# qinzheng93/GeoTransformer

Measured on NVIDIA H100. Metric: point-cloud pairs/sec (3DMatch-shape synth), higher is better.
Workload: dtype f32

## Files before the change

geotransformer_b200/csrc/evaluation.cu:

```cuda
#include "common.cuh"
#include "geob200.h"

namespace geob200 {

__device__ __forceinline__ float sqn3(float x, float y, float z) { return __fadd_rn(__fadd_rn(__fmul_rn(x, x), __fmul_rn(y, y)), __fmul_rn(z, z)); }
__device__ __forceinline__ float sqd_mm(float ax, float ay, float az, float a2, float bx, float by, float bz, float b2) {
    const float xy = fmaf(az, bz, fmaf(ay, by, __fmul_rn(ax, bx)));
    return fmaxf(__fadd_rn(__fsub_rn(a2, __fmul_rn(2.0f, xy)), b2), 0.0f);
}
__device__ __forceinline__ void xform(const float* T, float x, float y, float z, float& ox, float& oy, float& oz) {
    ox = fmaf(z, T[2], fmaf(y, T[1], x * T[0])) + T[3];
    oy = fmaf(z, T[6], fmaf(y, T[5], x * T[4])) + T[7];
    oz = fmaf(z, T[10], fmaf(y, T[9], x * T[8])) + T[11];
}

__global__ void __launch_bounds__(256) nc_prepare_kernel(const float* __restrict__ ref_nodes, const float* __restrict__ src_nodes,
                                                         const float* __restrict__ ref_knn_pts, const float* __restrict__ src_knn_pts,
                                                         const unsigned char* __restrict__ ref_knn_masks,
                                                         const unsigned char* __restrict__ src_knn_masks, const __grid_constant__ Segs cl,
                                                         int B, int K, const float* __restrict__ T, float* __restrict__ nodes_out,
                                                         float* __restrict__ pts_out, float* __restrict__ max_dist, int* __restrict__ n_valid) {
    const int lane = threadIdx.x & 31;
    const int s = blockIdx.y;
    const int m = blockIdx.x * 8 + (threadIdx.x >> 5);
// ... 26 lines not shown
#pragma unroll
    for (int o = 16; o > 0; o >>= 1) nv += __shfl_xor_sync(0xffffffffu, nv, o);
    if (lane == 0) {
        nodes_out[3 * m] = nx; nodes_out[3 * m + 1] = ny; nodes_out[3 * m + 2] = nz;
        max_dist[m] = md;
        n_valid[m] = nv;
    }
}

__global__ void __launch_bounds__(256) nc_overlap_kernel(const float* __restrict__ ref_nodes, const float* __restrict__ src_nodes,
                                                         const float* __restrict__ ref_pts, const float* __restrict__ src_pts,
                                                         const unsigned char* __restrict__ ref_knn_masks,
                                                         const unsigned char* __restrict__ src_knn_masks,
                                                         const unsigned char* __restrict__ ref_masks, const unsigned char* __restrict__ src_masks,
                                                         const float* __restrict__ ref_max, const float* __restrict__ src_max,
                                                         const int* __restrict__ ref_nv, const int* __restrict__ src_nv,
                                                         const __grid_constant__ Segs R, const __grid_constant__ Segs Q,
                                                         const __grid_constant__ Segs NN, int K, float pos_radius,
                                                         float* __restrict__ overlap ) {
    const int b = blockIdx.y;
    const int M = R.count[b], N = Q.count[b];
    if ((int)blockIdx.x >= M) return;
    {
        const long long r = R.start[b], q = Q.start[b];
        ref_nodes += 3 * r; ref_pts += 3 * r * K; ref_max += r; ref_nv += r;
        if (ref_knn_masks != nullptr) ref_knn_masks += r * K;
        if (ref_masks != nullptr) ref_masks += r;
        src_nodes += 3 * q; src_pts += 3 * q * K; src_max += q; src_nv += q;
        if (src_knn_masks != nullptr) src_knn_masks += q * K;
        if (src_masks != nullptr) src_masks += q;
        overlap += NN.start[b];
    }
    extern __shared__ float sm[];
    float4* rp = reinterpret_cast<float4*>(sm);
    float4* sp = rp + K;
    int* rhit = reinterpret_cast<int*>(sp + K);
    int* shit = rhit + K;
    __shared__ int tot[2];
    const int m = blockIdx.x;
    const float r2 = pos_radius * pos_radius;
    for (int i = threadIdx.x; i < K; i += blockDim.x) {
        const float* p = ref_pts + ((long long)m * K + i) * 3;
        const bool ok = ref_knn_masks == nullptr || ref_knn_masks[(long long)m * K + i];
        rp[i] = make_float4(p[0], p[1], p[2], ok ? sqn3(p[0], p[1], p[2]) : -1.f);
    }
    const bool m_ok = ref_masks == nullptr || ref_masks[m];
    const float mx = ref_nodes[3 * m], my = ref_nodes[3 * m + 1], mz = ref_nodes[3 * m + 2];
    const float m2 = sqn3(mx, my, mz);
    __syncthreads();
    for (int n = 0; n < N; ++n) {
        float ov = 0.f;
        const bool n_ok = src_masks == nullptr || src_masks[n];
        const float sx = src_nodes[3 * n], sy = src_nodes[3 * n + 1], sz = src_nodes[3 * n + 2];
        const float dist = sqrtf(sqd_mm(mx, my, mz, m2, sx, sy, sz, sqn3(sx, sy, sz)));
        const bool inter = m_ok && n_ok && (ref_max[m] + src_max[n] + pos_radius - dist > 0.f);
        if (inter) {
            for (int j = threadIdx.x; j < K; j += blockDim.x) {
                const float* p = src_pts + ((long long)n * K + j) * 3;
                const bool ok = src_knn_masks == nullptr || src_knn_masks[(long long)n * K + j];
                sp[j] = make_float4(p[0], p[1], p[2], ok ? sqn3(p[0], p[1], p[2]) : -1.f);
                shit[j] = 0;
                rhit[j] = 0;
            }
            __syncthreads();
            for (int e = threadIdx.x; e < K * K; e += blockDim.x) {
                const int i = e / K, j = e % K;
                const float4 a = rp[i], b = sp[j];
                if (a.w >= 0.f && b.w >= 0.f && sqd_mm(a.x, a.y, a.z, a.w, b.x, b.y, b.z, b.w) < r2) { rhit[i] = 1; shit[j] = 1; }
            }
            __syncthreads();
            int cr = 0, cs = 0;
            for (int i = threadIdx.x; i < K; i += blockDim.x) { cr += rhit[i]; cs += shit[i]; }
            if (threadIdx.x == 0) { tot[0] = 0; tot[1] = 0; }
            __syncthreads();
            if (cr) atomicAdd(&tot[0], cr);
            if (cs) atomicAdd(&tot[1], cs);
            __syncthreads();
            ov = ((float)tot[0] / (float)ref_nv[m] + (float)tot[1] / (float)src_nv[n]) / 2.0f;
            __syncthreads();
        }
        if (threadIdx.x == 0) overlap[(long long)m * N + n] = ov;
    }
}

__global__ void __launch_bounds__(1024) nc_compact_kernel(const float* __restrict__ overlap, const __grid_constant__ Segs R,
                                                          const __grid_constant__ Segs Q, const __grid_constant__ Segs NN,
                                                          long long* __restrict__ idx, float* __restrict__ ov_out, int* __restrict__ count) {
    const int b = blockIdx.x;
    const int M = R.count[b], N = Q.count[b];
    overlap += NN.start[b]; idx += 2ll * NN.start[b]; ov_out += NN.start[b]; count += b;
    __shared__ int warp_tot[32];
    __shared__ int carry;
    const int lane = threadIdx.x & 31, warp = threadIdx.x >> 5;
    if (threadIdx.x == 0) carry = 0;
    __syncthreads();
    const long long total = (long long)M * N;
    for (long long base = 0; base < total; base += 4096) {
        const long long t0 = base + 4ll * threadIdx.x;
        float v[4];
        int f = 0;
#pragma unroll
        for (int u = 0; u < 4; ++u) {
            v[u] = (t0 + u < total) ? overlap[t0 + u] : 0.f;
            f += v[u] > 0.f ? 1 : 0;
        }
        int incl = f;
#pragma unroll
        for (int o = 1; o < 32; o <<= 1) {
            const int y = __shfl_up_sync(0xffffffffu, incl, o);
            if (lane >= o) incl += y;
        }
        if (lane == 31) warp_tot[warp] = incl;
        __syncthreads();
        int off = carry + incl - f;
// ... 434 lines not shown

size_t geob200_node_correspondences_batched_workspace_bytes(int64_t n_rows, int64_t n_products, int64_t k) {
    const size_t r = (size_t)n_rows;
    return align_up(12 * r, 256) + align_up(12 * r * (size_t)k, 256) + 2 * align_up(4 * r, 256) + align_up(4 * (size_t)n_products, 256) + 256;
}

int geob200_node_correspondences_batched(const float* ref_nodes, const float* src_nodes, const float* ref_knn_points,
                                         const float* src_knn_points, const uint8_t* ref_masks, const uint8_t* src_masks,
                                         const uint8_t* ref_knn_masks, const uint8_t* src_knn_masks, int64_t n_pairs, const int64_t* cloud_nodes,
                                         int64_t k, const float* transforms, float pos_radius, int64_t* corr_indices, float* corr_overlaps,
                                         int32_t* count, void* workspace, size_t workspace_bytes, void* stream) {
    cudaStream_t st = (cudaStream_t)stream;
    GEOB_REQUIRE(n_pairs > 0 && 2 * n_pairs <= GEOB_MAX_CLOUDS, "node_correspondences_batched: 1..%d pairs", GEOB_MAX_CLOUDS / 2);
    GEOB_REQUIRE(k > 0 && k <= 1024, "node_correspondences: bad shape");
    const int B = (int)n_pairs;
    Segs cl, Q, NN;
    if (segs_from_counts(&cl, 2 * n_pairs, cloud_nodes) || segs_from_counts(&Q, n_pairs, cloud_nodes + n_pairs)) return -1;
    const Segs R = segs_range(cl, 0, B);
    const int64_t ref_rows = cl.start[B], rows = (int64_t)cl.start[2 * B - 1] + cl.count[2 * B - 1];
    GEOB_REQUIRE(ref_rows > 0 && rows > ref_rows, "node_correspondences: bad shape");
    if (segs_products(&NN, R, Q)) return -1;
    const int64_t nn = (int64_t)NN.start[B - 1] + NN.count[B - 1];
    GEOB_REQUIRE(workspace_bytes >= geob200_node_correspondences_batched_workspace_bytes(rows, nn, k),
                 "node_correspondences_batched: workspace too small");
    Arena ar(workspace, workspace_bytes);
    float* cn = ar.take<float>(3 * rows);
    float* cp = ar.take<float>(3 * rows * k);
    float* cmax = ar.take<float>(rows);
    int* cnv = ar.take<int>(rows);
    float* overlap = ar.take<float>(nn);
    GEOB_REQUIRE(ar.ok(), "node_correspondences: workspace accounting error");
    nc_prepare_kernel<<<dim3((unsigned)((cl.max + 7) / 8 > 0 ? (cl.max + 7) / 8 : 1), 2 * B), 256, 0, st>>>(
        ref_nodes, src_nodes, ref_knn_points, src_knn_points, ref_knn_masks, src_knn_masks, cl, B, (int)k, transforms, cn, cp, cmax, cnv);
    const size_t smem = (size_t)k * (2 * sizeof(float4) + 2 * sizeof(int));
    if (R.max > 0)
        nc_overlap_kernel<<<dim3((unsigned)R.max, B), 256, smem, st>>>(cn, cn + 3 * ref_rows, cp, cp + 3 * ref_rows * k, ref_knn_masks,
                                                                      src_knn_masks, ref_masks, src_masks, cmax, cmax + ref_rows, cnv,
                                                                      cnv + ref_rows, R, Q, NN, (int)k, pos_radius, overlap);
    nc_compact_kernel<<<B, 1024, 0, st>>>(overlap, R, Q, NN, (long long*)corr_indices, corr_overlaps, count);
    GEOB_CHECK_LAUNCH();
    count_launches(3);
    return 0;
}

static int evaluate_impl(const int64_t* gt_idx, const float* gt_ov, const Segs& G, const int32_t* n_gt_dev, float acceptance_overlap,
                         const int64_t* ref_idx, const int64_t* src_idx, int64_t n_node_corr, const int32_t* n_node_corr_dev,
                         const float* ref_pts, const float* src_pts, int64_t n_corr, const int32_t* n_corr_dev, float acceptance_radius,
                         const float* gt_transform, const float* est_transform, int64_t transform_ld, const float* src_points,
                         const Segs& S0, int mode, float rmse_threshold, float rre_threshold, float rte_threshold, float* metrics,
                         int64_t metrics_ld, cudaStream_t st) {
    GEOB_REQUIRE(mode >= 0 && mode <= 2, "evaluate: mode must be 0 (3DMatch), 1 (KITTI) or 2 (ModelNet)");
    evaluate_kernel<<<G.n, 1024, 0, st>>>((const long long*)gt_idx, gt_ov, G, acceptance_overlap, (const long long*)ref_idx,
                                          (const long long*)src_idx, (int)n_node_corr, ref_pts, src_pts, (int)n_corr, acceptance_radius,
                                          gt_transform, est_transform, (int)transform_ld, src_points, S0, mode, rmse_threshold, rre_threshold,
                                          rte_threshold, metrics, (int)metrics_ld, n_gt_dev, n_node_corr_dev, n_corr_dev);
    GEOB_CHECK_LAUNCH();
    count_launches(1);
    return 0;
}

int geob200_evaluate_counts(const int64_t* gt_node_corr_indices, const float* gt_node_corr_overlaps, int64_t n_gt, const int32_t* n_gt_dev,
                            float acceptance_overlap, const int64_t* ref_node_corr_indices, const int64_t* src_node_corr_indices,
                            int64_t n_node_corr, const int32_t* n_node_corr_dev, const float* ref_corr_points, const float* src_corr_points,
                            int64_t n_corr, const int32_t* n_corr_dev, float acceptance_radius, const float* gt_transform,
                            const float* est_transform, const float* src_points, int64_t n_src_points, int mode, float rmse_threshold,
                            float rre_threshold, float rte_threshold, float* metrics, void* stream) {
    return evaluate_impl(gt_node_corr_indices, gt_node_corr_overlaps, segs_one(n_gt), n_gt_dev, acceptance_overlap, ref_node_corr_indices,
// ... 223 lines not shown
```

geotransformer_b200/csrc/matching.cu:

```cuda
#include "common.cuh"
#include "geob200.h"

namespace geob200 {

int segs_from_counts(Segs* s, int64_t n, const int64_t* counts) {
    if (n < 1 || n > GEOB_MAX_CLOUDS) { set_error("batch: 1..%d segments supported (got %lld)", GEOB_MAX_CLOUDS, (long long)n); return -1; }
    *s = Segs{};
    s->n = (int)n;
    int64_t o = 0;
    for (int i = 0; i < n; ++i) {
        if (counts[i] < 0) { set_error("batch: negative segment size"); return -1; }
        s->start[i] = (int)o;
        s->count[i] = (int)counts[i];
        s->max = s->max > (int)counts[i] ? s->max : (int)counts[i];
        o += counts[i];
    }
    if (o >= (1ll << 31)) { set_error("batch: too many rows (%lld)", (long long)o); return -1; }
    return 0;
}

Segs segs_one(int64_t count) {
    Segs s{};
    s.n = 1;
    s.max = (int)count;
// ... 93 lines not shown
    }
}

__global__ void __launch_bounds__(256) spm_colsum_kernel(const float* __restrict__ S, const int* __restrict__ rcount,
                                                         const int* __restrict__ scount, const __grid_constant__ Segs Q,
                                                         const __grid_constant__ Segs NN, float* __restrict__ colsum) {
    const int p = blockIdx.y;
    const int ld = Q.count[p];
    S += NN.start[p]; rcount += p; scount += p; colsum += Q.start[p];
    const int j = blockIdx.x * blockDim.x + threadIdx.x;
    if (j >= *scount) return;
    const int nr = *rcount;
    float s = 0.f;
    for (int i = 0; i < nr; ++i) s += S[(long long)i * ld + j];
    colsum[j] = s;
}

__global__ void __launch_bounds__(256) spm_dual_kernel(const float* __restrict__ S, const int* __restrict__ rcount,
                                                       const int* __restrict__ scount, const float* __restrict__ rowsum,
                                                       const float* __restrict__ colsum, const __grid_constant__ Segs R,
                                                       const __grid_constant__ Segs Q, const __grid_constant__ Segs NN, int dual,
                                                       float* __restrict__ flat) {
    const int p = blockIdx.y;
    const int ld = Q.count[p];
    S += NN.start[p]; flat += NN.start[p]; rcount += p; scount += p; rowsum += R.start[p]; colsum += Q.start[p];
    const int nr = *rcount, ns = *scount;
    const long long t = (long long)blockIdx.x * blockDim.x + threadIdx.x;
    if (t >= (long long)nr * ns) return;
    const int i = (int)(t / ns), j = (int)(t % ns);
    const float v = S[(long long)i * ld + j];
    flat[t] = dual ? (v / rowsum[i]) * (v / colsum[j]) : v;
}

template <int KMAX>
__global__ void __launch_bounds__(1024) topk_flat_kernel(const float* __restrict__ flat, const int* __restrict__ rcount,
                                                         const int* __restrict__ scount, int k_req, const int* __restrict__ ridx,
                                                         const int* __restrict__ sidx, const __grid_constant__ Segs R,
                                                         const __grid_constant__ Segs Q, const __grid_constant__ Segs NN,
                                                         long long* __restrict__ ref_out, long long* __restrict__ src_out,
                                                         float* __restrict__ score_out, int* __restrict__ k_out) {
    {
        const int p = blockIdx.y;
        flat += NN.start[p]; rcount += p; scount += p; ridx += R.start[p]; sidx += Q.start[p];
        ref_out += (long long)p * k_req; src_out += (long long)p * k_req; score_out += (long long)p * k_req; k_out += p;
    }
    __shared__ unsigned hist[256];
    __shared__ unsigned long long keys[KMAX];
    __shared__ unsigned prefix_s, kth_s;
    __shared__ int warp_tot[32], carry_gt, carry_eq;
    const int nr = *rcount, ns = *scount;
    const long long total = (long long)nr * ns;
    const int k = (int)min((long long)min(k_req, KMAX), total);
    const int lane = threadIdx.x & 31, warp = threadIdx.x >> 5;
    for (int i = k + threadIdx.x; i < k_req; i += blockDim.x) { ref_out[i] = -1; src_out[i] = -1; score_out[i] = 0.f; }
    if (k == 0) { if (threadIdx.x == 0) *k_out = 0; return; }
    unsigned prefix = 0, mask = 0;
    int remaining = k;
    for (int shift = 24; shift >= 0; shift -= 8) {
        for (int i = threadIdx.x; i < 256; i += blockDim.x) hist[i] = 0;
        __syncthreads();
        for (long long t = threadIdx.x; t < total; t += blockDim.x) {
            const unsigned b = __float_as_uint(flat[t]);
            if ((b & mask) == prefix) atomicAdd(&hist[(b >> shift) & 255u], 1u);
        }
        __syncthreads();
        if (threadIdx.x == 0) {
            int rem = remaining;
            int d = 255;
            for (; d > 0; --d) {
                if ((int)hist[d] >= rem) break;
                rem -= (int)hist[d];
            }
            prefix_s = prefix | ((unsigned)d << shift);
            kth_s = (unsigned)rem;
        }
        __syncthreads();
        prefix = prefix_s;
        remaining = (int)kth_s;
        mask |= (255u << shift);
        __syncthreads();
    }
    const unsigned thr = prefix;
    const int need_eq = remaining;
    const int n_gt = k - need_eq;
    if (threadIdx.x == 0) { carry_gt = 0; carry_eq = 0; }
    __syncthreads();
    for (long long base = 0; base < total; base += 1024) {
        const long long t = base + threadIdx.x;
        unsigned b = 0;
        if (t < total) b = __float_as_uint(flat[t]);
        const int fg = (t < total && b > thr) ? 1 : 0;
        const int fe = (t < total && b == thr) ? 1 : 0;
        const unsigned bg = __ballot_sync(0xffffffffu, fg), be = __ballot_sync(0xffffffffu, fe);
        const int pg = __popc(bg & ((1u << lane) - 1u)), pe = __popc(be & ((1u << lane) - 1u));
        if (lane == 0) warp_tot[warp] = (__popc(bg) << 16) | __popc(be);
        __syncthreads();
        int og = carry_gt, oe = carry_eq;
        for (int w = 0; w < warp; ++w) { og += warp_tot[w] >> 16; oe += warp_tot[w] & 0xFFFF; }
        const unsigned long long key = ((unsigned long long)b << 32) | (unsigned)(0xFFFFFFFFu - (unsigned)t);
        if (fg) keys[og + pg] = key;
        if (fe && oe + pe < need_eq) keys[n_gt + oe + pe] = key;
        __syncthreads();
        if (threadIdx.x == 0) {
            int tg = 0, te = 0;
            for (int w = 0; w < 32; ++w) { tg += warp_tot[w] >> 16; te += warp_tot[w] & 0xFFFF; }
            carry_gt += tg; carry_eq += te;
        }
        __syncthreads();
    }
    int n2 = 1;
    while (n2 < k) n2 <<= 1;
    for (int i = k + threadIdx.x; i < n2; i += blockDim.x) keys[i] = 0ull;
    __syncthreads();
    for (int kk = 2; kk <= n2; kk <<= 1)
        for (int j = kk >> 1; j > 0; j >>= 1) {
            for (int t = threadIdx.x; t < n2; t += blockDim.x) {
                const int p = t ^ j;
                if (p > t) {
                    const unsigned long long a = keys[t], b = keys[p];
                    const bool desc = ((t & kk) == 0);
                    if ((a < b) == desc) { keys[t] = b; keys[p] = a; }
                }
            }
            __syncthreads();
        }
    for (int i = threadIdx.x; i < k; i += blockDim.x) {
        const unsigned long long key = keys[i];
        const unsigned t = 0xFFFFFFFFu - (unsigned)(key & 0xFFFFFFFFull);
        ref_out[i] = ridx[t / ns];
        src_out[i] = sidx[t % ns];
        score_out[i] = __uint_as_float((unsigned)(key >> 32));
    }
    if (threadIdx.x == 0) *k_out = k;
}

__global__ void __launch_bounds__(256) gather_patches_kernel(const long long* __restrict__ corr, int P_all, const long long* __restrict__ knn,
                                                             const unsigned char* __restrict__ knn_masks, int K,
                                                             const float* __restrict__ pts, const __grid_constant__ Segs Nd,
                                                             const __grid_constant__ Segs Pt, long long* __restrict__ out_idx,
                                                             unsigned char* __restrict__ out_mask, float* __restrict__ out_pts) {
    const int s = blockIdx.y;
    const int P = corr != nullptr ? P_all : Nd.count[s];
// ... 214 lines not shown
            }
#pragma unroll
            for (int o = LPR / 2; o > 0; o >>= 1) mx = fmaxf(mx, __shfl_xor_sync(0xffffffffu, mx, o));
            float s = 0.f;
#pragma unroll
            for (int k = 0; k < NE; ++k) s += exp2f(t[k] - mx);
#pragma unroll
            for (int o = LPR / 2; o > 0; o >>= 1) s += __shfl_xor_sync(0xffffffffu, s, o);
            if (act && sub == 0) u[ij] = lmu2 - (log2f(s) + mx);
        }
        __syncthreads();
        {
            float t[NE], mx = -INFINITY;
#pragma unroll
            for (int k = 0; k < NE; ++k) {
                const int o = sub + LPR * k;
                t[k] = zc[k] + u[o < K1 ? o : 0];
                mx = fmaxf(mx, t[k]);
            }
#pragma unroll
            for (int o = LPR / 2; o > 0; o >>= 1) mx = fmaxf(mx, __shfl_xor_sync(0xffffffffu, mx, o));
            float s = 0.f;
#pragma unroll
            for (int k = 0; k < NE; ++k) s += exp2f(t[k] - mx);
#pragma unroll
            for (int o = LPR / 2; o > 0; o >>= 1) s += __shfl_xor_sync(0xffffffffu, s, o);
            if (act && sub == 0) v[ij] = lnu2 - (log2f(s) + mx);
        }
        __syncthreads();
    }
    for (int e = threadIdx.x; e < K1 * K1; e += blockDim.x) {
        const int i = e / K1, j = e % K1;
        out[(long long)p * K1 * K1 + e] = Z[i * ld + j] + (u[i] + v[j]) * LN2 - norm;
    }
}

template <int K, int LPR, int MAXT, int MINB>
__global__ void __launch_bounds__(MAXT, MINB) sinkhorn_bwd_kernel(const float* __restrict__ scores, const unsigned char* __restrict__ row_masks,
                                                           const unsigned char* __restrict__ col_masks, const float* __restrict__ alpha_p,
                                                           int iters, float inf, const float* __restrict__ grad,
                                                           float* __restrict__ hist, float* __restrict__ dscores,
                                                           float* __restrict__ dalpha_part) {
    constexpr int K1 = K + 1, ld = K1 | 1, NE = (K1 + LPR - 1) / LPR;
    extern __shared__ float sm[];
    float* Z = sm;
    float* D = Z + K1 * ld;
    float* pu = D + K1 * ld;
    float* pv = pu + K1;
    float* Lu = pv + K1;
    float* Lv = Lu + K1;
    float* gu = Lv + K1;
    float* gv = gu + K1;
    unsigned char* rmk = reinterpret_cast<unsigned char*>(gv + K1);
    unsigned char* cmk = rmk + K1;
    __shared__ int cnt_s[2];
    const int p = blockIdx.x;
    row_masks += (long long)p * K; col_masks += (long long)p * K;
    grad += (long long)p * K1 * K1;
    hist += (long long)p * 2 * iters * K1;
    dscores += (long long)p * K * K;
    if (threadIdx.x < 2) cnt_s[threadIdx.x] = 0;
    __syncthreads();
    {
        int cr = 0, cc = 0;
        for (int i = threadIdx.x; i < K; i += blockDim.x) { cr += row_masks[i] ? 1 : 0; cc += col_masks[i] ? 1 : 0; }
        if (cr) atomicAdd(&cnt_s[0], cr);
// ... 294 lines not shown
                                                              const int* __restrict__ off, const int* __restrict__ keys,
                                                              int* __restrict__ sorted) {
    const long long e = (long long)blockIdx.x * blockDim.x + threadIdx.x;
    if (e >= 2 * pr.per_side) return;
    const int row = pr.row_of(e, R, Q);
    if (row < 0) return;
    const int b = off[row], n = off[row + 1] - b;
    int rank = 0;
    for (int s = 0; s < n; ++s) rank += keys[b + s] < (int)e;
    sorted[b + rank] = (int)e;
}

__global__ void __launch_bounds__(128) patch_rows_reduce_kernel(const float* __restrict__ tmp, int C, const int* __restrict__ off,
                                                                const int* __restrict__ sorted, int n_ref_rows, float* __restrict__ gref,
                                                                float* __restrict__ gsrc) {
    const int row = blockIdx.x;
    float* out = row < n_ref_rows ? gref + (long long)row * C : gsrc + (long long)(row - n_ref_rows) * C;
    const int b = off[row], n = off[row + 1] - b;
    for (int c = threadIdx.x; c < C; c += blockDim.x) {
        float s = 0.f;
        for (int k = 0; k < n; ++k) s += tmp[(long long)sorted[b + k] * C + c];
        out[c] = s;
    }
}

}

using namespace geob200;

extern "C" {

size_t geob200_superpoint_matching_batched_workspace_bytes(int64_t n_rows, int64_t n_products, int64_t n_pairs) {
    const size_t r = (size_t)n_rows, nn = (size_t)n_products;
    return align_up(4 * r, 256) * 3 + align_up(4 * nn, 256) * 2 + align_up(8 * (size_t)n_pairs, 256) + 4096;
}

int geob200_superpoint_matching_batched(const float* ref_feats, const float* src_feats, int64_t channels, const uint8_t* ref_masks,
                                        const uint8_t* src_masks, int64_t n_pairs, const int64_t* cloud_nodes, int64_t num_correspondences,
                                        int dual, int64_t* corr_indices, float* corr_scores, int32_t* num_out, void* workspace,
                                        size_t workspace_bytes, void* stream) {
    cudaStream_t st = (cudaStream_t)stream;
    GEOB_REQUIRE(n_pairs > 0 && 2 * n_pairs <= GEOB_MAX_CLOUDS, "superpoint_matching_batched: 1..%d pairs", GEOB_MAX_CLOUDS / 2);
    GEOB_REQUIRE(num_correspondences > 0 && num_correspondences <= 1024, "superpoint_matching: num_correspondences must be in 1..1024");
    const int B = (int)n_pairs;
    Segs cl, Q, NN;
    if (segs_from_counts(&cl, 2 * n_pairs, cloud_nodes) || segs_from_counts(&Q, n_pairs, cloud_nodes + n_pairs)) return -1;
    const Segs R = segs_range(cl, 0, B);
    const int64_t ref_rows = cl.start[B], rows = (int64_t)cl.start[2 * B - 1] + cl.count[2 * B - 1];
    GEOB_REQUIRE(ref_rows > 0 && rows > ref_rows, "superpoint_matching: empty input");
    if (segs_products(&NN, R, Q)) return -1;
    const int64_t nn = (int64_t)NN.start[B - 1] + NN.count[B - 1];
    GEOB_REQUIRE(workspace_bytes >= geob200_superpoint_matching_batched_workspace_bytes(rows, nn, n_pairs),
                 "superpoint_matching_batched: workspace too small");
    const size_t smem = sizeof(float) * (channels + Q.max);
    GEOB_REQUIRE(smem <= 48 * 1024, "superpoint_matching: row does not fit shared memory");
    Arena ar(workspace, workspace_bytes);
    int* idx = ar.take<int>(rows);
    float* rowsum = ar.take<float>(rows);
    float* colsum = ar.take<float>(rows);
    float* S = ar.take<float>(nn);
    float* flat = ar.take<float>(nn);
    int* counts = ar.take<int>(2 * B);
    const int* ridx = idx;
    const int* sidx = idx + ref_rows;
    const dim3 g_rows((unsigned)(R.max > 0 ? R.max : 1), B), g_cols((unsigned)((Q.max + 255) / 256 > 0 ? (Q.max + 255) / 256 : 1), B),
        g_nn((unsigned)((NN.max + 255) / 256 > 0 ? (NN.max + 255) / 256 : 1), B);
    const int64_t k = num_correspondences;
    compact_masks_kernel<<<dim3(1, 2 * B), 1024, 0, st>>>(ref_masks, src_masks, cl, B, idx, counts);
    spm_scores_kernel<<<g_rows, 256, smem, st>>>(ref_feats, src_feats, (int)channels, ridx, counts, sidx, counts + B, R, Q, NN, S, rowsum);
    spm_colsum_kernel<<<g_cols, 256, 0, st>>>(S, counts, counts + B, Q, NN, colsum);
    spm_dual_kernel<<<g_nn, 256, 0, st>>>(S, counts, counts + B, rowsum, colsum, R, Q, NN, dual, flat);
    topk_flat_kernel<1024><<<dim3(1, B), 1024, 0, st>>>(flat, counts, counts + B, (int)k, ridx, sidx, R, Q, NN, (long long*)corr_indices,
                                                        (long long*)corr_indices + B * k, corr_scores, num_out);
    GEOB_CHECK_LAUNCH();
    count_launches(5);
    return 0;
}

int geob200_gather_patches_batched(const int64_t* corr_indices, int64_t n_corr, int64_t n_clouds, const int64_t* cloud_nodes,
                                   const int64_t* cloud_points, const int64_t* node_knn_indices, const uint8_t* node_knn_masks, int64_t k,
                                   const float* points, int64_t* out_indices, uint8_t* out_masks, float* out_points, void* stream) {
    Segs nd, pt;
    if (segs_from_counts(&nd, n_clouds, cloud_nodes) || segs_from_counts(&pt, n_clouds, cloud_points)) return -1;
    const int64_t per = corr_indices != nullptr ? n_corr : nd.max;
    if (per == 0) return 0;
    gather_patches_kernel<<<dim3((unsigned)((per * k + 255) / 256), (unsigned)n_clouds), 256, 0, (cudaStream_t)stream>>>(
        (const long long*)corr_indices, (int)n_corr, (const long long*)node_knn_indices, node_knn_masks, (int)k, points, nd, pt,
        (long long*)out_indices, out_masks, out_points);
    GEOB_CHECK_LAUNCH();
    count_launches(1);
    return 0;
}

int geob200_patch_scores_batched(const float* ref_feats, const float* src_feats, int64_t channels, int64_t n_pairs, const int64_t* cloud_points,
                                 const int64_t* ref_knn_indices, const int64_t* src_knn_indices, int64_t n_patches, int64_t k,
                                 float* scores, void* stream) {
    cudaStream_t st = (cudaStream_t)stream;
    GEOB_REQUIRE(n_pairs > 0 && 2 * n_pairs <= GEOB_MAX_CLOUDS, "patch_scores_batched: 1..%d pairs", GEOB_MAX_CLOUDS / 2);
    Segs R, Q;
    if (segs_from_counts(&R, n_pairs, cloud_points) || segs_from_counts(&Q, n_pairs, cloud_points + n_pairs)) return -1;
    if (n_patches == 0) return 0;
    const float div = sqrtf((float)channels);
    const dim3 grid((unsigned)n_patches, R.n);
#define LAUNCH_PS(TV) patch_scores_kernel<TV><<<grid, 256, 0, st>>>(ref_feats, src_feats, R, Q, (int)channels,                      \
                                                                    (const long long*)ref_knn_indices, (const long long*)src_knn_indices, div, scores)
    if (k == 64) LAUNCH_PS(4);
    else if (k == 128) LAUNCH_PS(8);
    else if (k == 32) LAUNCH_PS(2);
    else
        GEOB_REQUIRE(false, "patch_scores: num_points_in_patch=%lld unsupported (32, 64, 128)", (long long)k);
#undef LAUNCH_PS
    GEOB_CHECK_LAUNCH();
    count_launches(1);
    return 0;
}

int geob200_sinkhorn(const float* scores, const uint8_t* row_masks, const uint8_t* col_masks, const float* alpha,
                     int64_t n_patches, int64_t k, int64_t num_iterations, float inf, float* out, void* stream) {
    cudaStream_t st = (cudaStream_t)stream;
    if (n_patches == 0) return 0;
    const int K1 = (int)k + 1, ld = K1 | 1;
    const size_t smem = sizeof(float) * ((size_t)K1 * ld + 4 * K1);
    GEOB_REQUIRE(smem <= 200 * 1024, "sinkhorn: patch too large (k=%lld)", (long long)k);
    if (smem > 48 * 1024 && ensure_max_smem((const void*)sinkhorn_kernel)) return -1;
#define LAUNCH_SK_REG(LPRV, NEV, MT)                                                                                                  \
    {                                                                                                                            \
        if (smem > 48 * 1024 && ensure_max_smem((const void*)sinkhorn_reg_kernel<LPRV, NEV, MT>)) return -1;                         \
        const int threads = ((K1 * LPRV + 31) / 32) * 32;                                                                        \
        sinkhorn_reg_kernel<LPRV, NEV, MT><<<(unsigned)n_patches, threads, smem, st>>>(scores, row_masks, col_masks, alpha, (int)k,  \
                                                                                  (int)num_iterations, inf, out);               \
    }
    if (K1 <= 40) LAUNCH_SK_REG(8, 5, 320)
    else if (K1 <= 72) LAUNCH_SK_REG(8, 9, 576)
    else if (K1 <= 132) LAUNCH_SK_REG(4, 33, 544)
    else
        sinkhorn_kernel<<<(unsigned)n_patches, 1024, smem, st>>>(scores, row_masks, col_masks, alpha, (int)k, (int)num_iterations, inf, out);
#undef LAUNCH_SK_REG
    GEOB_CHECK_LAUNCH();
    count_launches(1);
    return 0;
}

size_t geob200_sinkhorn_backward_workspace_bytes(int64_t n_patches, int64_t k, int64_t num_iterations) {
    const size_t K1 = (size_t)k + 1;
    return align_up(4 * (size_t)n_patches * 2 * (size_t)num_iterations * K1, 256) + align_up(4 * (size_t)n_patches, 256) + 256;
}

int geob200_sinkhorn_backward(const float* scores, const uint8_t* row_masks, const uint8_t* col_masks, const float* alpha, int64_t n_patches,
                              int64_t k, int64_t num_iterations, float inf, const float* grad_out, float* grad_scores, float* grad_alpha,
                              void* workspace, size_t workspace_bytes, void* stream) {
    cudaStream_t st = (cudaStream_t)stream;
    GEOB_REQUIRE(n_patches >= 0 && n_patches <= 0x7fffffff, "sinkhorn_backward: bad patch count");
    GEOB_REQUIRE(k == 32 || k == 64 || k == 128, "sinkhorn_backward: k must be 32, 64 or 128, got %lld", (long long)k);
    GEOB_REQUIRE(num_iterations >= 1 && num_iterations <= 100000, "sinkhorn_backward: num_iterations must be in 1..100000");
    GEOB_REQUIRE(inf > 0.f, "sinkhorn_backward: inf must be positive");
    GEOB_REQUIRE(scores != nullptr && row_masks != nullptr && col_masks != nullptr && alpha != nullptr && grad_out != nullptr &&
                     grad_scores != nullptr && grad_alpha != nullptr,
                 "sinkhorn_backward: null pointer");
    GEOB_REQUIRE(workspace_bytes >= geob200_sinkhorn_backward_workspace_bytes(n_patches, k, num_iterations),
                 "sinkhorn_backward: workspace too small");
    const int K1 = (int)k + 1, ld = K1 | 1;
    const size_t smem = sizeof(float) * (2 * (size_t)K1 * ld + 6 * K1) + 2 * (size_t)K1;
    Arena ar(workspace, workspace_bytes);
    float* hist = ar.take<float>((size_t)n_patches * 2 * num_iterations * K1);
    float* part = ar.take<float>((size_t)n_patches);
    GEOB_REQUIRE(ar.ok(), "sinkhorn_backward: workspace accounting error");
    int n_launch = 1;
    if (n_patches > 0) {
#define LAUNCH_SK_BWD(KV, LPRV, MT, MB)                                                                                               \
    {                                                                                                                                 \
// ... 88 lines not shown
```

Measured before the change: 437.5.

## Warp-per-pair overlap, two-stage chunked top-k, and register Sinkhorn variant

Three independent changes. The node-overlap kernel now gives each warp its own source node, with per-warp shared buffers and ballot/popc reductions replacing block-wide syncs and shared atomics. Superpoint top-k becomes two stages: per-chunk radix selection of candidates across many blocks, then a final single-block select over the candidates, instead of one block scanning all scores. A new Sinkhorn kernel for small patches spreads each line over 8 lanes holding two lines per group, using ex2.approx, and needs more workspace and shared memory.

```diff
diff --git a/geotransformer_b200/csrc/evaluation.cu b/geotransformer_b200/csrc/evaluation.cu
--- a/geotransformer_b200/csrc/evaluation.cu
+++ b/geotransformer_b200/csrc/evaluation.cu
@@ -82,11 +82,9 @@
         overlap += NN.start[b];
     }
     extern __shared__ float sm[];
+    const int lane = threadIdx.x & 31, warp = threadIdx.x >> 5, nw = blockDim.x >> 5;
     float4* rp = reinterpret_cast<float4*>(sm);
-    float4* sp = rp + K;
-    int* rhit = reinterpret_cast<int*>(sp + K);
-    int* shit = rhit + K;
-    __shared__ int tot[2];
+    float4* sp = rp + K + warp * K;
     const int m = blockIdx.x;
     const float r2 = pos_radius * pos_radius;
     for (int i = threadIdx.x; i < K; i += blockDim.x) {
@@ -98,38 +96,37 @@
     const float mx = ref_nodes[3 * m], my = ref_nodes[3 * m + 1], mz = ref_nodes[3 * m + 2];
     const float m2 = sqn3(mx, my, mz);
     __syncthreads();
-    for (int n = 0; n < N; ++n) {
+    for (int n = warp; n < N; n += nw) {
         float ov = 0.f;
         const bool n_ok = src_masks == nullptr || src_masks[n];
         const float sx = src_nodes[3 * n], sy = src_nodes[3 * n + 1], sz = src_nodes[3 * n + 2];
         const float dist = sqrtf(sqd_mm(mx, my, mz, m2, sx, sy, sz, sqn3(sx, sy, sz)));
         const bool inter = m_ok && n_ok && (ref_max[m] + src_max[n] + pos_radius - dist > 0.f);
         if (inter) {
-            for (int j = threadIdx.x; j < K; j += blockDim.x) {
+            for (int j = lane; j < K; j += 32) {
                 const float* p = src_pts + ((long long)n * K + j) * 3;
                 const bool ok = src_knn_masks == nullptr || src_knn_masks[(long long)n * K + j];
                 sp[j] = make_float4(p[0], p[1], p[2], ok ? sqn3(p[0], p[1], p[2]) : -1.f);
-                shit[j] = 0;
-                rhit[j] = 0;
             }
-            __syncthreads();
-            for (int e = threadIdx.x; e < K * K; e += blockDim.x) {
-                const int i = e / K, j = e % K;
-                const float4 a = rp[i], b = sp[j];
-                if (a.w >= 0.f && b.w >= 0.f && sqd_mm(a.x, a.y, a.z, a.w, b.x, b.y, b.z, b.w) < r2) { rhit[i] = 1; shit[j] = 1; }
+            __syncwarp();
+            unsigned rhit = 0;
+            int cs = 0;
+            for (int j = 0; j < K; ++j) {
+                const float4 b = sp[j];
+                bool hit = false;
+                for (int q = 0, i = lane; i < K; ++q, i += 32) {
+                    const float4 a = rp[i];
+                    if (a.w >= 0.f && b.w >= 0.f && sqd_mm(a.x, a.y, a.z, a.w, b.x, b.y, b.z, b.w) < r2) { rhit |= 1u << q; hit = true; }
+                }
+                cs += __any_sync(0xffffffffu, hit) ? 1 : 0;
             }
-            __syncthreads();
-            int cr = 0, cs = 0;
-            for (int i = threadIdx.x; i < K; i += blockDim.x) { cr += rhit[i]; cs += shit[i]; }
-            if (threadIdx.x == 0) { tot[0] = 0; tot[1] = 0; }
-            __syncthreads();
-            if (cr) atomicAdd(&tot[0], cr);
-            if (cs) atomicAdd(&tot[1], cs);
-            __syncthreads();
-            ov = ((float)tot[0] / (float)ref_nv[m] + (float)tot[1] / (float)src_nv[n]) / 2.0f;
-            __syncthreads();
-        }
-        if (threadIdx.x == 0) overlap[(long long)m * N + n] = ov;
+            int cr = __popc(rhit);
+#pragma unroll
+            for (int o = 16; o > 0; o >>= 1) cr += __shfl_xor_sync(0xffffffffu, cr, o);
+            ov = ((float)cr / (float)ref_nv[m] + (float)cs / (float)src_nv[n]) / 2.0f;
+            __syncwarp();
+        }
+        if (lane == 0) overlap[(long long)m * N + n] = ov;
     }
 }
 
@@ -630,7 +627,8 @@
     GEOB_REQUIRE(ar.ok(), "node_correspondences: workspace accounting error");
     nc_prepare_kernel<<<dim3((unsigned)((cl.max + 7) / 8 > 0 ? (cl.max + 7) / 8 : 1), 2 * B), 256, 0, st>>>(
         ref_nodes, src_nodes, ref_knn_points, src_knn_points, ref_knn_masks, src_knn_masks, cl, B, (int)k, transforms, cn, cp, cmax, cnv);
-    const size_t smem = (size_t)k * (2 * sizeof(float4) + 2 * sizeof(int));
+    const size_t smem = (size_t)k * sizeof(float4) * (1 + 256 / 32);
+    if (smem > 48 * 1024 && ensure_max_smem((const void*)nc_overlap_kernel)) return -1;
     if (R.max > 0)
         nc_overlap_kernel<<<dim3((unsigned)R.max, B), 256, smem, st>>>(cn, cn + 3 * ref_rows, cp, cp + 3 * ref_rows * k, ref_knn_masks,
                                                                       src_knn_masks, ref_masks, src_masks, cmax, cmax + ref_rows, cnv,
diff --git a/geotransformer_b200/csrc/matching.cu b/geotransformer_b200/csrc/matching.cu
--- a/geotransformer_b200/csrc/matching.cu
+++ b/geotransformer_b200/csrc/matching.cu
@@ -149,82 +149,131 @@
     flat[t] = dual ? (v / rowsum[i]) * (v / colsum[j]) : v;
 }
 
-template <int KMAX>
-__global__ void __launch_bounds__(1024) topk_flat_kernel(const float* __restrict__ flat, const int* __restrict__ rcount,
-                                                         const int* __restrict__ scount, int k_req, const int* __restrict__ ridx,
-                                                         const int* __restrict__ sidx, const __grid_constant__ Segs R,
-                                                         const __grid_constant__ Segs Q, const __grid_constant__ Segs NN,
-                                                         long long* __restrict__ ref_out, long long* __restrict__ src_out,
-                                                         float* __restrict__ score_out, int* __restrict__ k_out) {
-    {
-        const int p = blockIdx.y;
-        flat += NN.start[p]; rcount += p; scount += p; ridx += R.start[p]; sidx += Q.start[p];
-        ref_out += (long long)p * k_req; src_out += (long long)p * k_req; score_out += (long long)p * k_req; k_out += p;
-    }
-    __shared__ unsigned hist[256];
-    __shared__ unsigned long long keys[KMAX];
-    __shared__ unsigned prefix_s, kth_s;
-    __shared__ int warp_tot[32], carry_gt, carry_eq;
-    const int nr = *rcount, ns = *scount;
-    const long long total = (long long)nr * ns;
-    const int k = (int)min((long long)min(k_req, KMAX), total);
-    const int lane = threadIdx.x & 31, warp = threadIdx.x >> 5;
-    for (int i = k + threadIdx.x; i < k_req; i += blockDim.x) { ref_out[i] = -1; src_out[i] = -1; score_out[i] = 0.f; }
-    if (k == 0) { if (threadIdx.x == 0) *k_out = 0; return; }
+constexpr int TOPK_CHUNK = 4096;
+constexpr int TOPK_KMAX = 1024;
+
+struct TopkShared {
+    unsigned hist[256];
+    unsigned prefix, kth;
+    int warp_tot[32], carry_gt, carry_eq;
+};
+
+template <typename Get>
+__device__ __forceinline__ void topk_threshold(int n, int k, Get b_of, TopkShared& sh, unsigned& thr, int& need_eq) {
     unsigned prefix = 0, mask = 0;
     int remaining = k;
     for (int shift = 24; shift >= 0; shift -= 8) {
-        for (int i = threadIdx.x; i < 256; i += blockDim.x) hist[i] = 0;
-        __syncthreads();
-        for (long long t = threadIdx.x; t < total; t += blockDim.x) {
-            const unsigned b = __float_as_uint(flat[t]);
-            if ((b & mask) == prefix) atomicAdd(&hist[(b >> shift) & 255u], 1u);
+        for (int i = threadIdx.x; i < 256; i += blockDim.x) sh.hist[i] = 0;
+        __syncthreads();
+        for (int t = threadIdx.x; t < n; t += blockDim.x) {
+            const unsigned b = b_of(t);
+            if ((b & mask) == prefix) atomicAdd(&sh.hist[(b >> shift) & 255u], 1u);
         }
         __syncthreads();
         if (threadIdx.x == 0) {
             int rem = remaining;
             int d = 255;
             for (; d > 0; --d) {
-                if ((int)hist[d] >= rem) break;
-                rem -= (int)hist[d];
+                if ((int)sh.hist[d] >= rem) break;
+                rem -= (int)sh.hist[d];
             }
-            prefix_s = prefix | ((unsigned)d << shift);
-            kth_s = (unsigned)rem;
-        }
-        __syncthreads();
-        prefix = prefix_s;
-        remaining = (int)kth_s;
+            sh.prefix = prefix | ((unsigned)d << shift);
+            sh.kth = (unsigned)rem;
+        }
+        __syncthreads();
+        prefix = sh.prefix;
+        remaining = (int)sh.kth;
         mask |= (255u << shift);
         __syncthreads();
     }
-    const unsigned thr = prefix;
-    const int need_eq = remaining;
-    const int n_gt = k - need_eq;
-    if (threadIdx.x == 0) { carry_gt = 0; carry_eq = 0; }
-    __syncthreads();
-    for (long long base = 0; base < total; base += 1024) {
-        const long long t = base + threadIdx.x;
-        unsigned b = 0;
-        if (t < total) b = __float_as_uint(flat[t]);
-        const int fg = (t < total && b > thr) ? 1 : 0;
-        const int fe = (t < total && b == thr) ? 1 : 0;
+    thr = prefix;
+    need_eq = remaining;
+}
+
+template <typename Get, typename Emit>
+__device__ __forceinline__ void topk_sweep(int n, unsigned thr, int need_eq, Get b_of, TopkShared& sh, Emit emit) {
+    const int lane = threadIdx.x & 31, warp = threadIdx.x >> 5, nw = blockDim.x >> 5;
+    if (threadIdx.x == 0) { sh.carry_gt = 0; sh.carry_eq = 0; }
+    __syncthreads();
+    for (int base = 0; base < n; base += blockDim.x) {
+        const int t = base + threadIdx.x;
+        const unsigned b = t < n ? b_of(t) : 0u;
+        const int fg = (t < n && b > thr) ? 1 : 0;
+        const int fe = (t < n && b == thr) ? 1 : 0;
         const unsigned bg = __ballot_sync(0xffffffffu, fg), be = __ballot_sync(0xffffffffu, fe);
         const int pg = __popc(bg & ((1u << lane) - 1u)), pe = __popc(be & ((1u << lane) - 1u));
-        if (lane == 0) warp_tot[warp] = (__popc(bg) << 16) | __popc(be);
-        __syncthreads();
-        int og = carry_gt, oe = carry_eq;
-        for (int w = 0; w < warp; ++w) { og += warp_tot[w] >> 16; oe += warp_tot[w] & 0xFFFF; }
-        const unsigned long long key = ((unsigned long long)b << 32) | (unsigned)(0xFFFFFFFFu - (unsigned)t);
-        if (fg) keys[og + pg] = key;
-        if (fe && oe + pe < need_eq) keys[n_gt + oe + pe] = key;
+        if (lane == 0) sh.warp_tot[warp] = (__popc(bg) << 16) | __popc(be);
+        __syncthreads();
+        int og = sh.carry_gt, oe = sh.carry_eq;
+        for (int w = 0; w < warp; ++w) { og += sh.warp_tot[w] >> 16; oe += sh.warp_tot[w] & 0xFFFF; }
+        if (fg || (fe && oe + pe < need_eq)) emit(og + pg + min(oe + pe, need_eq), t, b);
         __syncthreads();
         if (threadIdx.x == 0) {
             int tg = 0, te = 0;
-            for (int w = 0; w < 32; ++w) { tg += warp_tot[w] >> 16; te += warp_tot[w] & 0xFFFF; }
-            carry_gt += tg; carry_eq += te;
-        }
-        __syncthreads();
-    }
+            for (int w = 0; w < nw; ++w) { tg += sh.warp_tot[w] >> 16; te += sh.warp_tot[w] & 0xFFFF; }
+            sh.carry_gt += tg; sh.carry_eq += te;
+        }
+        __syncthreads();
+    }
+}
+
+__global__ void __launch_bounds__(256) topk_chunk_kernel(const float* __restrict__ flat, const int* __restrict__ rcount,
+                                                         const int* __restrict__ scount, int k_req, const __grid_constant__ Segs NN,
+                                                         unsigned* __restrict__ cand_b, unsigned* __restrict__ cand_t) {
+    const int p = blockIdx.y, c = blockIdx.x;
+    const long long total = (long long)rcount[p] * scount[p];
+    const int k = (int)min((long long)min(k_req, TOPK_KMAX), total);
+    const long long first = (long long)c * TOPK_CHUNK;
+    if (first >= total) return;
+    const int n = (int)min((long long)TOPK_CHUNK, total - first);
+    flat += NN.start[p] + first;
+    const long long slot = ((long long)NN.start[p] / TOPK_CHUNK + p + c) * k_req;
+    cand_b += slot; cand_t += slot;
+    __shared__ unsigned vals[TOPK_CHUNK];
+    __shared__ TopkShared sh;
+    for (int i = threadIdx.x; i < n; i += blockDim.x) vals[i] = __float_as_uint(flat[i]);
+    if (n <= k) {
+        for (int i = threadIdx.x; i < n; i += blockDim.x) { cand_b[i] = vals[i]; cand_t[i] = (unsigned)(first + i); }
+        return;
+    }
+    __syncthreads();
+    const auto b_of = [&](int t) { return vals[t]; };
+    unsigned thr;
+    int need_eq;
+    topk_threshold(n, k, b_of, sh, thr, need_eq);
+    topk_sweep(n, thr, need_eq, b_of, sh, [&](int slot, int t, unsigned b) { cand_b[slot] = b; cand_t[slot] = (unsigned)(first + t); });
+}
+
+template <int KMAX>
+__global__ void __launch_bounds__(1024) topk_flat_kernel(const unsigned* __restrict__ cand_b, const unsigned* __restrict__ cand_t,
+                                                         const int* __restrict__ rcount, const int* __restrict__ scount, int k_req,
+                                                         const int* __restrict__ ridx, const int* __restrict__ sidx,
+                                                         const __grid_constant__ Segs R, const __grid_constant__ Segs Q,
+                                                         const __grid_constant__ Segs NN, long long* __restrict__ ref_out,
+                                                         long long* __restrict__ src_out, float* __restrict__ score_out,
+                                                         int* __restrict__ k_out) {
+    {
+        const int p = blockIdx.y;
+        const long long slot = ((long long)NN.start[p] / TOPK_CHUNK + p) * k_req;
+        cand_b += slot; cand_t += slot; rcount += p; scount += p; ridx += R.start[p]; sidx += Q.start[p];
+        ref_out += (long long)p * k_req; src_out += (long long)p * k_req; score_out += (long long)p * k_req; k_out += p;
+    }
+    __shared__ unsigned long long keys[KMAX];
+    __shared__ TopkShared sh;
+    const int nr = *rcount, ns = *scount;
+    const long long total = (long long)nr * ns;
+    const int k = (int)min((long long)min(k_req, KMAX), total);
+    for (int i = k + threadIdx.x; i < k_req; i += blockDim.x) { ref_out[i] = -1; src_out[i] = -1; score_out[i] = 0.f; }
+    if (k == 0) { if (threadIdx.x == 0) *k_out = 0; return; }
+    const long long chunks = (total + TOPK_CHUNK - 1) / TOPK_CHUNK;
+    const int n = (int)((chunks - 1) * k_req + min((long long)k, total - (chunks - 1) * TOPK_CHUNK));
+    const auto b_of = [&](int t) { return cand_b[t]; };
+    unsigned thr;
+    int need_eq;
+    topk_threshold(n, k, b_of, sh, thr, need_eq);
+    topk_sweep(n, thr, need_eq, b_of, sh, [&](int slot, int t, unsigned b) {
+        keys[slot] = ((unsigned long long)b << 32) | (unsigned)(0xFFFFFFFFu - cand_t[t]);
+    });
     int n2 = 1;
     while (n2 < k) n2 <<= 1;
     for (int i = k + threadIdx.x; i < n2; i += blockDim.x) keys[i] = 0ull;
@@ -505,6 +554,158 @@
     for (int e = threadIdx.x; e < K1 * K1; e += blockDim.x) {
         const int i = e / K1, j = e % K1;
         out[(long long)p * K1 * K1 + e] = Z[i * ld + j] + (u[i] + v[j]) * LN2 - norm;
+    }
+}
+
+__device__ __forceinline__ float ex2_ftz(float x) {
+    float y;
+    asm("ex2.approx.ftz.f32 %0, %1;" : "=f"(y) : "f"(x));
+    return y;
+}
+
+template <int NE>
+struct SkLines {
+    static constexpr int PS = ((NE + 3) / 4 * 4) | 4;
+    static constexpr int ZS = ((2 * NE + 3) / 4 * 4) % 8 ? (2 * NE + 3) / 4 * 4 : (2 * NE + 3) / 4 * 4 + 4;
+};
+
+template <int NE, int NL>
+__device__ __forceinline__ void sinkhorn2_half_step(const float (&z)[2][NE], const float* __restrict__ pin, float* __restrict__ pout,
+                                                    int sub, const int (&line)[2], const bool (&own)[2], const float (&marg)[2]) {
+    constexpr int PS = SkLines<NE>::PS;
+    constexpr float LOG2E = 1.4426950408889634f;
+    float pv[NE];
+    {
+        const float* src = pin + sub * PS;
+#pragma unroll
+        for (int k = 0; k + 4 <= NE; k += 4) {
+            const float4 q = *reinterpret_cast<const float4*>(src + k);
+            pv[k] = q.x; pv[k + 1] = q.y; pv[k + 2] = q.z; pv[k + 3] = q.w;
+        }
+#pragma unroll
+        for (int k = NE / 4 * 4; k < NE; ++k) pv[k] = src[k];
+    }
+    float t[NL][NE], mx[NL], s[NL];
+#pragma unroll
+    for (int l = 0; l < NL; ++l) {
+        mx[l] = -INFINITY;
+#pragma unroll
+        for (int k = 0; k < NE; ++k) {
+            t[l][k] = __fadd_rn(z[l][k], pv[k]);
+            mx[l] = fmaxf(mx[l], t[l][k]);
+        }
+    }
+#pragma unroll
+    for (int o = 4; o > 0; o >>= 1)
+#pragma unroll
+        for (int l = 0; l < NL; ++l) mx[l] = fmaxf(mx[l], __shfl_xor_sync(0xffffffffu, mx[l], o));
+#pragma unroll
+    for (int l = 0; l < NL; ++l) {
+        s[l] = ex2_ftz(__fsub_rn(t[l][0], mx[l]));
+#pragma unroll
+        for (int k = 1; k < NE; ++k) s[l] = __fadd_rn(s[l], ex2_ftz(__fsub_rn(t[l][k], mx[l])));
+    }
+#pragma unroll
+    for (int o = 4; o > 0; o >>= 1)
+#pragma unroll
+        for (int l = 0; l < NL; ++l) s[l] = __fadd_rn(s[l], __shfl_xor_sync(0xffffffffu, s[l], o));
+    const bool second = NL == 2 && sub == 1;
+    if (sub < NL && (second ? own[1] : own[0])) {
+        const float ss = second ? s[NL - 1] : s[0], m = second ? mx[NL - 1] : mx[0];
+        const int i = second ? line[1] : line[0];
+        pout[(i & 7) * PS + (i >> 3)] = __fmaf_rn(second ? marg[1] : marg[0], LOG2E, -(log2f(ss) + m));
+    }
+}
+
+template <int NE, int MAXT, int MINB>
+__global__ void __launch_bounds__(MAXT, MINB) sinkhorn_reg2_kernel(const float* __restrict__ scores, const unsigned char* __restrict__ row_masks,
+                                                                   const unsigned char* __restrict__ col_masks, const float* __restrict__ alpha_p,
+                                                                   int K, int iters, float inf, float* __restrict__ out) {
+    constexpr int PS = SkLines<NE>::PS, ZS = SkLines<NE>::ZS;
+    extern __shared__ float sm[];
+    __shared__ __align__(16) float up[8 * PS], vp[8 * PS];
+    __shared__ float norm_s;
+    __shared__ int cnt_s[2];
+    const int K1 = K + 1;
+    const int ld = K1 | 1;
+    const int H = (K1 + 1) >> 1;
+    float* Z = sm;
+    float* zcs = sm + ((K1 * ld + 3) & ~3) + threadIdx.x * ZS;
+    const int p = blockIdx.x;
+    const float alpha = *alpha_p;
+    constexpr float LOG2E = 1.4426950408889634f, LN2 = 0.6931471805599453f;
+    if (threadIdx.x < 2) cnt_s[threadIdx.x] = 0;
+    for (int i = threadIdx.x; i < 8 * PS; i += blockDim.x) { up[i] = 0.f; vp[i] = 0.f; }
+    __syncthreads();
+    {
+        int cr = 0, cc = 0;
+        for (int i = threadIdx.x; i < K; i += blockDim.x) { cr += row_masks[(long long)p * K + i] ? 1 : 0; cc += col_masks[(long long)p * K + i] ? 1 : 0; }
+        if (cr) atomicAdd(&cnt_s[0], cr);
+        if (cc) atomicAdd(&cnt_s[1], cc);
+    }
+    __syncthreads();
+    const float nvr = (float)cnt_s[0], nvc = (float)cnt_s[1];
+    if (threadIdx.x == 0) norm_s = -logf(nvr + nvc);
+    __syncthreads();
+    const float norm = norm_s;
+    for (int e = threadIdx.x; e < K1 * K1; e += blockDim.x) {
+        const int i = e / K1, j = e % K1;
+        float z = (i < K && j < K) ? scores[((long long)p * K + i) * K + j] : alpha;
+        const bool rm = (i < K) && !row_masks[(long long)p * K + i];
+        const bool cm = (j < K) && !col_masks[(long long)p * K + j];
+        if (rm || cm) z = -inf;
+        Z[i * ld + j] = z;
+    }
+    __syncthreads();
+    const int g = threadIdx.x >> 3, sub = threadIdx.x & 7;
+    const bool two = ((threadIdx.x >> 5) << 2) + H < K1;
+    int line[2];
+    bool own[2];
+    float zr[2][NE], mu[2], nu[2];
+#pragma unroll
+    for (int l = 0; l < 2; ++l) {
+        const int i = g + l * H;
+        own[l] = (l == 0 ? g < H : true) && i < K1;
+        line[l] = own[l] ? i : K1 - 1;
+        const int ij = line[l];
+#pragma unroll
+        for (int k = 0; k < NE; ++k) {
+            const int o = sub + 8 * k;
+            zr[l][k] = (o < K1) ? __fmul_rn(Z[ij * ld + o], LOG2E) : -INFINITY;
+            zcs[l * NE + k] = (o < K1) ? __fmul_rn(Z[o * ld + ij], LOG2E) : -INFINITY;
+        }
+        float m = (ij < K) ? norm : logf(nvc) + norm;
+        float n = (ij < K) ? norm : logf(nvr) + norm;
+        if (ij < K && !row_masks[(long long)p * K + ij]) m = -inf;
+        if (ij < K && !col_masks[(long long)p * K + ij]) n = -inf;
+        mu[l] = m;
+        nu[l] = n;
+    }
+    for (int it = 0; it < iters; ++it) {
+        if (two) sinkhorn2_half_step<NE, 2>(zr, vp, up, sub, line, own, mu);
+        else sinkhorn2_half_step<NE, 1>(zr, vp, up, sub, line, own, mu);
+        __syncthreads();
+        float zc[2][NE];
+        {
+            float buf[ZS];
+#pragma unroll
+            for (int q = 0; q < ZS; q += 4) {
+                const float4 v4 = *reinterpret_cast<const float4*>(zcs + q);
+                buf[q] = v4.x; buf[q + 1] = v4.y; buf[q + 2] = v4.z; buf[q + 3] = v4.w;
+            }
+#pragma unroll
+            for (int l = 0; l < 2; ++l)
+#pragma unroll
+                for (int k = 0; k < NE; ++k) zc[l][k] = buf[l * NE + k];
+        }
+        if (two) sinkhorn2_half_step<NE, 2>(zc, up, vp, sub, line, own, nu);
+        else sinkhorn2_half_step<NE, 1>(zc, up, vp, sub, line, own, nu);
+        __syncthreads();
+    }
+    for (int e = threadIdx.x; e < K1 * K1; e += blockDim.x) {
+        const int i = e / K1, j = e % K1;
+        const float uv = __fadd_rn(up[(i & 7) * PS + (i >> 3)], vp[(j & 7) * PS + (j >> 3)]);
+        out[(long long)p * K1 * K1 + e] = __fsub_rn(__fmaf_rn(uv, LN2, Z[i * ld + j]), norm);
     }
 }
 
@@ -865,7 +1066,8 @@
 
 size_t geob200_superpoint_matching_batched_workspace_bytes(int64_t n_rows, int64_t n_products, int64_t n_pairs) {
     const size_t r = (size_t)n_rows, nn = (size_t)n_products;
-    return align_up(4 * r, 256) * 3 + align_up(4 * nn, 256) * 2 + align_up(8 * (size_t)n_pairs, 256) + 4096;
+    const size_t cand = (nn / TOPK_CHUNK + (size_t)n_pairs) * TOPK_KMAX;
+    return align_up(4 * r, 256) * 3 + align_up(4 * nn, 256) * 2 + align_up(8 * (size_t)n_pairs, 256) + 2 * align_up(4 * cand, 256) + 4096;
 }
 
 int geob200_superpoint_matching_batched(const float* ref_feats, const float* src_feats, int64_t channels, const uint8_t* ref_masks,
@@ -894,6 +1096,9 @@
     float* S = ar.take<float>(nn);
     float* flat = ar.take<float>(nn);
     int* counts = ar.take<int>(2 * B);
+    const size_t n_cand = ((size_t)nn / TOPK_CHUNK + (size_t)B) * TOPK_KMAX;
+    unsigned* cand_b = ar.take<unsigned>(n_cand);
+    unsigned* cand_t = ar.take<unsigned>(n_cand);
     const int* ridx = idx;
     const int* sidx = idx + ref_rows;
     const dim3 g_rows((unsigned)(R.max > 0 ? R.max : 1), B), g_cols((unsigned)((Q.max + 255) / 256 > 0 ? (Q.max + 255) / 256 : 1), B),
@@ -903,10 +1108,12 @@
     spm_scores_kernel<<<g_rows, 256, smem, st>>>(ref_feats, src_feats, (int)channels, ridx, counts, sidx, counts + B, R, Q, NN, S, rowsum);
     spm_colsum_kernel<<<g_cols, 256, 0, st>>>(S, counts, counts + B, Q, NN, colsum);
     spm_dual_kernel<<<g_nn, 256, 0, st>>>(S, counts, counts + B, rowsum, colsum, R, Q, NN, dual, flat);
-    topk_flat_kernel<1024><<<dim3(1, B), 1024, 0, st>>>(flat, counts, counts + B, (int)k, ridx, sidx, R, Q, NN, (long long*)corr_indices,
-                                                        (long long*)corr_indices + B * k, corr_scores, num_out);
+    topk_chunk_kernel<<<dim3((unsigned)((NN.max + TOPK_CHUNK - 1) / TOPK_CHUNK > 0 ? (NN.max + TOPK_CHUNK - 1) / TOPK_CHUNK : 1), B), 256, 0,
+                        st>>>(flat, counts, counts + B, (int)k, NN, cand_b, cand_t);
+    topk_flat_kernel<TOPK_KMAX><<<dim3(1, B), 1024, 0, st>>>(cand_b, cand_t, counts, counts + B, (int)k, ridx, sidx, R, Q, NN,
+                                                             (long long*)corr_indices, (long long*)corr_indices + B * k, corr_scores, num_out);
     GEOB_CHECK_LAUNCH();
-    count_launches(5);
+    count_launches(6);
     return 0;
 }
 
@@ -963,12 +1170,21 @@
         sinkhorn_reg_kernel<LPRV, NEV, MT><<<(unsigned)n_patches, threads, smem, st>>>(scores, row_masks, col_masks, alpha, (int)k,  \
                                                                                   (int)num_iterations, inf, out);               \
     }
-    if (K1 <= 40) LAUNCH_SK_REG(8, 5, 320)
-    else if (K1 <= 72) LAUNCH_SK_REG(8, 9, 576)
+#define LAUNCH_SK_REG2(NEV, MT, MB)                                                                                                  \
+    {                                                                                                                            \
+        const int threads = (((K1 + 1) / 2 * 8 + 31) / 32) * 32;                                                                 \
+        const size_t smem2 = sizeof(float) * ((((size_t)K1 * ld + 3) & ~(size_t)3) + (size_t)threads * SkLines<NEV>::ZS);     \
+        if (smem2 > 48 * 1024 && ensure_max_smem((const void*)sinkhorn_reg2_kernel<NEV, MT, MB>)) return -1;                       \
+        sinkhorn_reg2_kernel<NEV, MT, MB><<<(unsigned)n_patches, threads, smem2, st>>>(scores, row_masks, col_masks, alpha, (int)k, \
+                                                                                 (int)num_iterations, inf, out);              \
+    }
+    if (K1 <= 40) LAUNCH_SK_REG2(5, 160, 4)
+    else if (K1 <= 72) LAUNCH_SK_REG2(9, 288, 4)
     else if (K1 <= 132) LAUNCH_SK_REG(4, 33, 544)
     else
         sinkhorn_kernel<<<(unsigned)n_patches, 1024, smem, st>>>(scores, row_masks, col_masks, alpha, (int)k, (int)num_iterations, inf, out);
 #undef LAUNCH_SK_REG
+#undef LAUNCH_SK_REG2
     GEOB_CHECK_LAUNCH();
     count_launches(1);
     return 0;
```

Result: faster. 466.7, median of 6 (+6.7%).
